# georgeretsi/smirk

Hardware: AMD Instinct MI355X
Metric: faces/sec (encode+FLAME+render+generate) @224x224 (higher is better)
Workload: dtype f32 results; encoder + generator convs as split-fp16 x3 MFMA with f32 accumulate (fp32-class error), FLAME / raster f32

## Files before the change

include/smirk_hip.h:

```cpp
#ifndef SMIRK_HIP_H
#define SMIRK_HIP_H

#include <stddef.h>
#include <stdint.h>

#ifdef __cplusplus
extern "C" {
#endif

#define SMIRK_OK 0
#define SMIRK_ERR_BAD_ARG (-1)
#define SMIRK_ERR_WORKSPACE (-2)
#define SMIRK_ERR_LAUNCH (-3)
#define SMIRK_ERR_UNSUPPORTED (-4)

const char* smirk_strerror(int code);
unsigned smirk_range_flag_peek(void);
void smirk_range_flag_clear(void);

int smirk_abi_version(void);

#define SMIRK_FLAME_KCHUNK 32

typedef struct SmirkFlameModel {
// ... 115 lines not shown
int smirk_pack_generator_input_split16(const float* a, int Ca, const float* b, int Cb, void* out, int B, int H, int W, void* stream);
int smirk_conv1x1_sigmoid_nchw_split16(const void* in, const float* w , const float* bias, float* out,
                                       int B, int H, int W, int C, int Cout, void* stream);

int smirk_maxpool2x2_nhwc(const float* in, float* out, int B, int H, int W, int C, void* stream);
int smirk_nchw_to_nhwc_pad(const float* in, float* out, int B, int Cin, int H, int W, int Cpad, void* stream);
int smirk_pack_generator_input(const float* rendered, const float* masked, float* out, int B, int H, int W, void* stream);
int smirk_conv1x1_sigmoid_nchw(const float* in, const float* w , const float* bias, float* out,
                               int B, int H, int W, int C, int Cout, void* stream);

int smirk_stem_conv_s2(const float* img_nchw, const float* w , const float* scale,
                       const float* shift, float* out, int B, int H, int W, int Cout, void* stream);
int smirk_dwconv3x3(const float* in, const float* w , const float* scale, const float* shift, float* out,
                    int B, int H, int W, int C, int stride, int relu, void* stream);
int smirk_gap_linear(const float* feat, const float* w, const float* bias, float* out, float* ws, int B, int HW, int C, int N,
                     void* stream);
int smirk_stem_conv_s2_split16(const float* img_nchw, const float* w, const float* scale, const float* shift, void* out, int B, int H,
                               int W, int Cout, void* stream);
int smirk_dwconv3x3_split16(const void* in, const float* w , const float* scale, const float* shift, void* out, int B, int H,
                            int W, int C, int stride, int relu, void* stream);
int smirk_gap_linear_split16(const void* feat, const float* w, const float* bias, float* out, float* ws, int B, int HW, int C, int N,
                             void* stream);
int smirk_expression_clamps(float* params, int B, int n_exp, void* stream);

int smirk_mask_face_weights(const float* tverts, const float* normals, const int32_t* faces , const float* face_prob ,
                            int B, int V, int F, float* weights , void* stream);
int smirk_sample_faces(const float* weights, int B, int F, int num, uint64_t seed, uint64_t offset, int32_t* idx, float* bary,
                       void* stream);
int smirk_points_to_pixels(const float* points, int B, int L, int image_size, int64_t* out, void* stream);
int smirk_maxpool_sq(const float* in, float* tmp, float* out, int B, int H, int W, int radius, int complement, void* stream);
int smirk_bernoulli_field(float* out, size_t n, float p, uint64_t seed, uint64_t offset, void* stream);
int smirk_masking_compose(const float* img, const float* mask, const float* rendered_mask, const float* extra_points ,
                          const float* pmask ,
                          const float* keep, const float* noise_mult, int B, int C, int H, int W, int gen_noise,
                          uint64_t seed, uint64_t offset, float* out, void* stream);
int smirk_rendered_mask(const float* rendered_img, int B, int C, int H, int W, float* out, void* stream);
int smirk_scatter_points_mask(const int64_t* points, const int64_t* rbound, int B, int L, int H, int W, float* out, void* stream);
int smirk_transfer_pixels(const float* img, const int64_t* points1, const int64_t* points2, const int64_t* rbound, int B, int C,
                          int L, int H, int W, int32_t* winner_ws, float* out, void* stream);

size_t smirk_mbconv_lds_bytes(int Cin, int mid, int Cout, int stride);
int smirk_mbconv_image_supported(int H, int W, int Cin, int mid, int Cout, int stride);
int smirk_mbconv_image_split16(const void* x, const void* wexp, const float* s1, const float* b1, const float* wdw, const float* s2, const float* b2,
                               const void* wproj, const float* s3, const float* b3, int residual, void* out, int B, int H, int W, int Cin, int mid,
                               int Cout, void* stream);
int smirk_encoder_head_supported(int stem_cout, int kind, int cin, int mid, int cout, int stride, int skip);
int smirk_encoder_head_fused_split16(const float* img, const float* stem_w, const float* stem_scale, const float* stem_shift, const float* dw_w,
                                     const float* dw_scale, const float* dw_shift, const void* pw_w, const float* pw_scale, const float* pw_shift,
                                     int residual, void* out, int B, int H, int W, int stride, void* stream);
int smirk_mbconv_supported(int Cin, int mid, int Cout, int stride);
int smirk_mbconv_fused_split16(const void* x, const void* wexp, const float* s1, const float* b1, const float* wdw, const float* s2,
                               const float* b2, const void* wproj, const float* s3, const float* b3, int residual, void* out,
                               int B, int H, int W, int Cin, int mid, int Cout, int stride, void* stream);

typedef struct SmirkConvLayer {
    const void* w;
    const float* scale;
    const float* shift;
} SmirkConvLayer;

#define SMIRK_GEN_MAX_RES 16
enum { SMIRK_PRECISION_F32 = 0, SMIRK_PRECISION_F16X3 = 1 };

typedef struct SmirkGeneratorWeights {
    int32_t in_channels, out_channels, features, res_blocks;
    int32_t precision;
    int32_t cin_pad;
    SmirkConvLayer enc[5][2];
    SmirkConvLayer res[SMIRK_GEN_MAX_RES][2];
    SmirkConvLayer up[4];
    SmirkConvLayer dec[4][2];
    const float* final_w;
    const float* final_b;
} SmirkGeneratorWeights;

size_t smirk_generator_workspace_bytes(const SmirkGeneratorWeights* w , int B, int H, int W);
int smirk_generator_forward(const SmirkGeneratorWeights* w, const float* a, int Ca, const float* b, int Cb, float* y,
                            int B, int H, int W, void* const* taps, void* ws, size_t ws_bytes, void* stream);

typedef struct SmirkMbBlock {
    int32_t kind, stride, cin, mid, cout, skip;
    SmirkConvLayer pw, dw, pwl;
} SmirkMbBlock;

#define SMIRK_BACKBONE_MAX_BLOCKS 24
typedef struct SmirkBackboneWeights {
    int32_t n_blocks, precision, n_out;
    int32_t clamp_n_exp;
    int32_t stem_cout, feat_ch;
    SmirkConvLayer stem;
    SmirkMbBlock blocks[SMIRK_BACKBONE_MAX_BLOCKS];
    const float* head_w;
    const float* head_b;
} SmirkBackboneWeights;

size_t smirk_backbone_workspace_bytes(const SmirkBackboneWeights* w , int B, int H, int W);
int smirk_backbone_forward(const SmirkBackboneWeights* w, const float* img, int B, int H, int W, float* out, void* feat_out,
                           void* ws, size_t ws_bytes, void* stream);

size_t smirk_train_reduce_workspace_bytes(int C);
int smirk_bn_train_forward_split16(const void* z, size_t M, int C, const float* gamma, const float* beta, const void* residual, int relu, float eps,
                                   float momentum, float* running_mean, float* running_var, long long* num_batches_tracked, float* save_mean,
                                   float* save_var, float* save_invstd, void* y, void* ws, size_t ws_bytes, void* stream);
size_t smirk_conv_stats_rows_max(const SmirkConvDesc* d);
int smirk_conv_igemm_stats_split16(const SmirkConvDesc* d, const void* in0, const void* in1, const void* w, void* out, float* stats, int* rows, int x1, void* stream);
int smirk_bn_train_forward_partials_split16(const void* z, size_t M, int C, const float* gamma, const float* beta, const void* residual, int relu, float eps,
// ... 98 lines not shown
```

smirk_amd/_lib.py:

```python
import ctypes as C
import os

import torch

HERE = os.path.dirname(os.path.abspath(__file__))
LIB_PATH = os.path.join(HERE, "lib", "libsmirk_hip.so")
LIB_PATH = os.environ.get("SMIRK_HIP_LIBRARY", LIB_PATH)
ABI_VERSION = 13
PACK_DEPTHWISE, PACK_STEM, PACK_CONVT2X2 = -3, -27, -2
SMIRK_OK, SMIRK_ERR_BAD_ARG, SMIRK_ERR_WORKSPACE, SMIRK_ERR_LAUNCH, SMIRK_ERR_UNSUPPORTED = 0, -1, -2, -3, -4

_p = C.c_void_p
_i = C.c_int
_sz = C.c_size_t


class SmirkFlameModel(C.Structure):
    _fields_ = [(n, C.c_int32) for n in ("V", "VP", "F", "n_shape", "n_exp", "KP", "n_static", "n_dyn", "n_lut",
                                         "n_full", "n_mp", "_pad")] + \
               [(n, _p) for n in ("dirs", "v_template", "lbs_weights", "jdirs", "jtemplate", "l_eyelid", "r_eyelid",
                                  "faces", "static_faces", "static_bary", "dyn_faces", "dyn_bary", "full_faces",
                                  "full_bary", "mp_faces", "mp_bary")]


class SmirkRenderMesh(C.Structure):
    _fields_ = [(n, C.c_int32) for n in ("V", "Vf", "Ff", "nnz")] + \
               [(n, _p) for n in ("keep", "faces", "nrm_ptr", "nrm_face", "nrm_corner")]


class SmirkConvDesc(C.Structure):
    _fields_ = [(n, C.c_int32) for n in ("B", "H", "W", "C0", "C1", "Cout", "KH", "KW", "stride", "pad_t", "pad_l",
                                         "Ho", "Wo", "pad_mode", "act", "out_mode")]


class SmirkConvLayer(C.Structure):
    _fields_ = [("w", _p), ("scale", _p), ("shift", _p)]


GEN_MAX_RES, BACKBONE_MAX_BLOCKS = 16, 24
PRECISION_F32, PRECISION_F16X3 = 0, 1


class SmirkGeneratorWeights(C.Structure):
    _fields_ = [(n, C.c_int32) for n in ("in_channels", "out_channels", "features", "res_blocks", "precision", "cin_pad")] + \
               [("enc", SmirkConvLayer * 2 * 5), ("res", SmirkConvLayer * 2 * GEN_MAX_RES), ("up", SmirkConvLayer * 4),
                ("dec", SmirkConvLayer * 2 * 4), ("final_w", _p), ("final_b", _p)]


class SmirkMbBlock(C.Structure):
    _fields_ = [(n, C.c_int32) for n in ("kind", "stride", "cin", "mid", "cout", "skip")] + \
               [("pw", SmirkConvLayer), ("dw", SmirkConvLayer), ("pwl", SmirkConvLayer)]


class SmirkBackboneWeights(C.Structure):
    _fields_ = [(n, C.c_int32) for n in ("n_blocks", "precision", "n_out", "clamp_n_exp", "stem_cout", "feat_ch")] + \
               [("stem", SmirkConvLayer), ("blocks", SmirkMbBlock * BACKBONE_MAX_BLOCKS), ("head_w", _p), ("head_b", _p)]


class SmirkProfileRecord(C.Structure):
    _fields_ = [("kernel", C.c_char * 120), ("flop", C.c_double), ("bytes", C.c_double), ("ms", C.c_float), ("_pad", C.c_int32)]


LOSS_MAX_TERMS, LOSS_CHUNK = 8, 4096
LOSS_SQUARE, LOSS_ABS_IMAGE = 0, 1


class SmirkLossTerm(C.Structure):
    _fields_ = [("pred", _p), ("target", _p), ("row_flags", _p)] + \
               [(n, C.c_int32) for n in ("rows", "row_stride", "cols", "kind", "C", "HW")] + \
               [("weight", C.c_float), ("loss_img", _p), ("grad", _p)]


PAD_ZERO, PAD_REFLECT = 0, 1
ACT_NONE, ACT_RELU = 0, 1
OUT_NHWC, OUT_CONVT2X2 = 0, 1

_SIGS = {
    "smirk_strerror": (C.c_char_p, [_i]),
    "smirk_abi_version": (_i, []),
    "smirk_range_flag_peek": (C.c_uint, []),
    "smirk_range_flag_clear": (None, []),
    "smirk_flame_workspace_bytes": (_sz, [C.POINTER(SmirkFlameModel), _i]),
    "smirk_flame_forward": (_i, [C.POINTER(SmirkFlameModel), _i, _p, _i, _p, _i, _p, _p, _p, _p, _p, _p, _p, _p, _p, _p,
                                 _p, _p, _sz, _p]),
    "smirk_flame_backward_workspace_bytes": (_sz, [C.POINTER(SmirkFlameModel), _i]),
    "smirk_flame_backward": (_i, [C.POINTER(SmirkFlameModel), _p, _i, _p, _i, _p, _i] + [_p] * 5 + [_p, _p] + [_p] * 4 + [_p] * 7 +
                             [_p, _sz, _p]),
    "smirk_vertices2landmarks": (_i, [_p, _i, _i, _p, _p, _p, _i, _p, _p]),
    "smirk_render_workspace_bytes": (_sz, [C.POINTER(SmirkRenderMesh), _i, _i, _i]),
    "smirk_render_forward": (_i, [C.POINTER(SmirkRenderMesh), _i, _i, _i, _p, _p, _p, _p, _p, _p, _p, _p, _p, _sz, _p]),
    "smirk_vertex_normals": (_i, [C.POINTER(SmirkRenderMesh), _i, _p, _p, _p]),
    "smirk_mask_face_weights": (_i, [_p, _p, _p, _p, _i, _i, _i, _p, _p]),
    "smirk_sample_faces": (_i, [_p, _i, _i, _i, C.c_uint64, C.c_uint64, _p, _p, _p]),
    "smirk_points_to_pixels": (_i, [_p, _i, _i, _i, _p, _p]),
    "smirk_maxpool_sq": (_i, [_p, _p, _p, _i, _i, _i, _i, _i, _p]),
    "smirk_bernoulli_field": (_i, [_p, _sz, C.c_float, C.c_uint64, C.c_uint64, _p]),
    "smirk_masking_compose": (_i, [_p, _p, _p, _p, _p, _p, _p, _i, _i, _i, _i, _i, C.c_uint64, C.c_uint64, _p, _p]),
    "smirk_render_backward_workspace_bytes": (_sz, [C.POINTER(SmirkRenderMesh), _i, _i, _i]),
    "smirk_render_backward": (_i, [C.POINTER(SmirkRenderMesh), _i, _i, _i, _p, _p, _p, _p, _p, _p, _p, _p, _sz, _p]),
    "smirk_project_landmarks_backward": (_i, [_p, _p, _p, _i, _i, _p, _p, _p]),
    "smirk_encoder_head_supported": (_i, [_i] * 7),
    "smirk_encoder_head_fused_split16": (_i, [_p] * 10 + [_i, _p] + [_i] * 4 + [_p]),
    "smirk_mbconv_image_supported": (_i, [_i] * 6),
    "smirk_mbconv_image_split16": (_i, [_p] * 10 + [_i, _p] + [_i] * 6 + [_p]),
    "smirk_mbconv_lds_bytes": (_sz, [_i, _i, _i, _i]),
    "smirk_mbconv_supported": (_i, [_i, _i, _i, _i]),
    "smirk_mbconv_fused_split16": (_i, [_p] * 10 + [_i, _p] + [_i] * 7 + [_p]),
    "smirk_warp_affine_u8": (_i, [_p, _i, _i, _i, _p, _i, _i, _i, _p, _p, _p]),
    "smirk_resize_linear_u8": (_i, [_p, _i, _i, _i, _i, _i, _i, _p, _p, _p]),
    "smirk_f32_nchw_to_u8_grid": (_i, [_p, _i, _i, _i, _i, _p, _i, _i, _p]),
    "smirk_u8_hwc_to_f32_nchw": (_i, [_p, _i, _i, _i, _i, _p, _p]),
    "smirk_interp_bilinear_f32": (_i, [_p, _i, _i, _i, _i, _i, _p, _p]),
    "smirk_hull_mask": (_i, [_p, _i, _i, _i, _i, _i, _p, _p]),
    "smirk_rendered_mask": (_i, [_p, _i, _i, _i, _i, _p, _p]),
    "smirk_scatter_points_mask": (_i, [_p, _p, _i, _i, _i, _i, _p, _p]),
    "smirk_transfer_pixels": (_i, [_p, _p, _p, _p, _i, _i, _i, _i, _i, _p, _p, _p]),
    "smirk_project_landmarks": (_i, [_p, _p, _i, _i, _p, _p]),
    "smirk_conv_igemm_f32": (_i, [C.POINTER(SmirkConvDesc), _p, _p, _p, _p, _p, _p, _p, _p]),
    "smirk_conv_igemm_f16x3": (_i, [C.POINTER(SmirkConvDesc), _p, _p, _p, _p, _p, _p, _p, _p]),
    "smirk_conv_igemm_f16x1": (_i, [C.POINTER(SmirkConvDesc), _p, _p, _p, _p, _p, _p, _p, _p]),
    "smirk_conv3x3_tail_f16x3": (_i, [C.POINTER(SmirkConvDesc), _p, _p, _p, _p, _p, _p, _p, _p, _i, _p]),
    "smirk_conv3x3_pool_f16x3": (_i, [C.POINTER(SmirkConvDesc), _p, _p, _p, _p, _p, _p, _p, _p]),
    "smirk_enc1_fused_supported": (_i, [_i, _i, _i, _i]),
    "smirk_enc1_fused_split16": (_i, [_p] * 9 + [_i, _i, _i, _p]),
    "smirk_f32_to_split16": (_i, [_p, _p, _sz, _p]),
    "smirk_split16_to_f32": (_i, [_p, _p, _sz, _p]),
    "smirk_maxpool2x2_split16": (_i, [_p, _p, _i, _i, _i, _i, _p]),
    "smirk_split16_range_check": (_i, [_p, _sz, C.c_float, _p, _p]),
    "smirk_pack_generator_input_split16": (_i, [_p, _i, _p, _i, _p, _i, _i, _i, _p]),
    "smirk_conv1x1_sigmoid_nchw_split16": (_i, [_p, _p, _p, _p, _i, _i, _i, _i, _i, _p]),
    "smirk_maxpool2x2_nhwc": (_i, [_p, _p, _i, _i, _i, _i, _p]),
    "smirk_nchw_to_nhwc_pad": (_i, [_p, _p, _i, _i, _i, _i, _i, _p]),
    "smirk_pack_generator_input": (_i, [_p, _p, _p, _i, _i, _i, _p]),
    "smirk_conv1x1_sigmoid_nchw": (_i, [_p, _p, _p, _p, _i, _i, _i, _i, _i, _p]),
    "smirk_stem_conv_s2": (_i, [_p, _p, _p, _p, _p, _i, _i, _i, _i, _p]),
    "smirk_dwconv3x3": (_i, [_p, _p, _p, _p, _p, _i, _i, _i, _i, _i, _i, _p]),
    "smirk_gap_linear": (_i, [_p, _p, _p, _p, _p, _i, _i, _i, _i, _p]),
    "smirk_stem_conv_s2_split16": (_i, [_p, _p, _p, _p, _p, _i, _i, _i, _i, _p]),
    "smirk_dwconv3x3_split16": (_i, [_p, _p, _p, _p, _p, _i, _i, _i, _i, _i, _i, _p]),
    "smirk_gap_linear_split16": (_i, [_p, _p, _p, _p, _p, _i, _i, _i, _i, _p]),
    "smirk_expression_clamps": (_i, [_p, _i, _i, _p]),
    "smirk_generator_workspace_bytes": (_sz, [C.POINTER(SmirkGeneratorWeights), _i, _i, _i]),
    "smirk_generator_forward": (_i, [C.POINTER(SmirkGeneratorWeights), _p, _i, _p, _i, _p, _i, _i, _i, C.POINTER(_p), _p, _sz, _p]),
    "smirk_backbone_workspace_bytes": (_sz, [C.POINTER(SmirkBackboneWeights), _i, _i, _i]),
    "smirk_backbone_forward": (_i, [C.POINTER(SmirkBackboneWeights), _p, _i, _i, _i, _p, _p, _p, _sz, _p]),
    "smirk_train_reduce_workspace_bytes": (_sz, [_i]),
    "smirk_conv_stats_rows_max": (_sz, [C.POINTER(SmirkConvDesc)]),
    "smirk_conv_igemm_stats_split16": (_i, [C.POINTER(SmirkConvDesc), _p, _p, _p, _p, _p, C.POINTER(C.c_int), _i, _p]),
    "smirk_bn_train_forward_partials_split16": (_i, [_p, _sz, _i, _p, _p, _p, _i, C.c_float, C.c_float, _p, _p, _p, _p, _p, _p, _p, _p, _i, _i, _p]),
    "smirk_dwconv3x3_stats_split16": (_i, [_p, _p, _p, _i, _i, _i, _i, _i, _p, C.POINTER(C.c_int), _p]),
    "smirk_bn_train_forward_split16": (_i, [_p, _sz, _i, _p, _p, _p, _i, C.c_float, C.c_float, _p, _p, _p, _p, _p, _p, _p, _p, _sz, _p]),
    "smirk_bn_train_backward_split16": (_i, [_p, _p, _sz, _i, _p, _p, _p, _p, _i, _p, _p, _p, _p, _sz, _p]),
    "smirk_bn_eval_forward_split16": (_i, [_p, _sz, _i, _p, _p, _p, _p, _p, _i, C.c_float, _p, _p, _p, _p]),
    "smirk_bn_eval_backward_split16": (_i, [_p, _p, _sz, _i, _p, _p, _p, _p, _p, _i, _p, _p]),
    "smirk_colsum_split16": (_i, [_p, _sz, _i, _p, _p, _sz, _p]),
    "smirk_maxpool2x2_backward_split16": (_i, [_p, _p, _p, _p, _i, _i, _i, _i, _p]),
    "smirk_reflect_pad1_backward_split16": (_i, [_p, _p, _p, _i, _i, _i, _i, _p]),
    "smirk_space_to_depth2_split16": (_i, [_p, _p, _i, _i, _i, _i, _p]),
    "smirk_conv1x1_sigmoid_backward_split16": (_i, [_p, _p, _p, _p, _p, _i, _i, _i, _i, _i, _p]),
    "smirk_conv_wgrad_set_mode": (_i, [_i]),
# ... 149 lines not shown
```

smirk_amd/csrc/capi.hip:

```cpp
#include <stdlib.h>
#include <string.h>

#include <map>
#include <mutex>
#include <utility>
#include <vector>

#include "common.h"

extern "C" const char* smirk_strerror(int code) {
    switch (code) {
        case SMIRK_OK: return "ok";
        case SMIRK_ERR_BAD_ARG: return "bad argument (null pointer, size or alignment constraint violated)";
        case SMIRK_ERR_WORKSPACE: return "workspace too small (see smirk_*_workspace_bytes)";
        case SMIRK_ERR_LAUNCH: return "HIP kernel launch failed";
        case SMIRK_ERR_UNSUPPORTED: return "configuration not supported by the gfx950 kernels";
        default: return "unknown smirk error";
    }
}

extern "C" int smirk_abi_version(void) { return 13; }

int smirk_switch(SmirkSwitch s) {
    static const char* const names[] = {"SMIRK_IGEMM_HALO", "SMIRK_IGEMM_PP", "SMIRK_CONV_RING", "SMIRK_DISABLE_PATCH_KERNEL", "SMIRK_DISABLE_ENC1_FUSED",
                                        "SMIRK_DISABLE_MBCONV_IMAGE", "SMIRK_DISABLE_MBCONV_TILE", "SMIRK_DISABLE_MBCONV_FUSED",
                                        "SMIRK_DISABLE_ENCODER_HEAD_FUSED", "SMIRK_GEN_SPLIT_CHAINS", "SMIRK_WGRAD_F16"};
    static_assert(sizeof(names) / sizeof(names[0]) == SMIRK_SW_COUNT, "one name per SmirkSwitch");
    const char* e = getenv(names[s]);
    switch (s) {
        case SMIRK_SW_IGEMM_HALO:
        case SMIRK_SW_CONV_RING: return !e || e[0] != '0';
        case SMIRK_SW_IGEMM_PP: return !e ? 1 : e[0] == '0' ? 0 : e[0] == 'a' ? 2 : 1;
        case SMIRK_SW_GEN_SPLIT_CHAINS: return !e ? 0 : e[0] == '0' ? 1 : e[0] == '3' ? 3 : 2;
        case SMIRK_SW_WGRAD_F16: return e ? atoi(e) : SMIRK_WGRAD_F16_DEFAULT;
        default: return e != nullptr;
    }
}

namespace {
std::mutex g_dev_mu;
std::map<std::pair<int, const void*>, size_t> g_lds_raised;
std::map<int, int> g_dev_cus;
}

int smirk_raise_dynamic_lds(const void* kernel, size_t bytes) {
    int dev = 0;
    if (hipGetDevice(&dev) != hipSuccess) { (void)hipGetLastError(); return SMIRK_ERR_LAUNCH; }
    std::lock_guard<std::mutex> lk(g_dev_mu);
    size_t& raised = g_lds_raised[{dev, kernel}];
    if (bytes <= raised) return SMIRK_OK;
    if (hipFuncSetAttribute(kernel, hipFuncAttributeMaxDynamicSharedMemorySize, (int)bytes) != hipSuccess) { (void)hipGetLastError(); return SMIRK_ERR_LAUNCH; }
    raised = bytes;
    return SMIRK_OK;
}

int smirk_device_cus() {
    int dev = 0;
    if (hipGetDevice(&dev) != hipSuccess) { (void)hipGetLastError(); return 256; }
    std::lock_guard<std::mutex> lk(g_dev_mu);
    auto it = g_dev_cus.find(dev);
    if (it != g_dev_cus.end()) return it->second;
    int cus = 0;
    if (hipDeviceGetAttribute(&cus, hipDeviceAttributeMultiprocessorCount, dev) != hipSuccess || cus <= 0) { (void)hipGetLastError(); cus = 256; }
    g_dev_cus[dev] = cus;
    return cus;
}

namespace {
std::once_flag g_range_once;
unsigned* g_range_host = nullptr;
unsigned* g_range_dev = nullptr;
}
unsigned* smirk_range_flag_device_ptr() {
    std::call_once(g_range_once, [] {
// ... 85 lines not shown
```

smirk_amd/csrc/network.hip:

```cpp
#include <sys/syscall.h>
#include <unistd.h>
#include <stdlib.h>

#include "common.h"

namespace {

struct Arena {
    char* base;
    size_t off;
    void* take(size_t bytes) {
        off = smirk_align_up(off, 256);
        void* p = base ? base + off : nullptr;
        off += bytes;
        return p;
    }
};

struct Rot {
    void* slot[3];
    void* pick(const void* a, const void* b) const {
        for (int i = 0; i < 3; ++i)
            if (slot[i] != a && slot[i] != b) return slot[i];
        return nullptr;
    }
};

inline size_t act_bytes(int B, int H, int W, int C) { return (size_t)B * H * W * C * 4; }

struct GenPlan {
    void* x;
    void* e[4];
    Rot rot;
    size_t total;
};

GenPlan plan_generator(const SmirkGeneratorWeights* w, int B, int H, int W, void* ws) {
    Arena a{(char*)ws, 0};
    GenPlan p;
    const int f = w->features;
    p.x = a.take(act_bytes(B, H, W, w->cin_pad));
    for (int l = 0; l < 4; ++l) p.e[l] = a.take(act_bytes(B, H >> l, W >> l, f << l));
    const size_t big = act_bytes(B, H, W, f);
    for (int i = 0; i < 3; ++i) p.rot.slot[i] = a.take(big);
    p.total = smirk_align_up(a.off, 256);
    return p;
}

int conv_call(bool split, const SmirkConvDesc& d, const void* in0, const void* in1, const SmirkConvLayer& L, const void* residual, void* out,
              void* stream) {
    return split ? smirk_conv_igemm_f16x3(&d, in0, in1, L.w, L.scale, L.shift, residual, out, stream)
                 : smirk_conv_igemm_f32(&d, (const float*)in0, (const float*)in1, (const float*)L.w, L.scale, L.shift, (const float*)residual,
                                        (float*)out, stream);
}

SmirkConvDesc desc3x3(int B, int H, int W, int c0, int c1, int cout, bool reflect, bool relu) {
    SmirkConvDesc d;
// ... 284 lines not shown
extern "C" size_t smirk_backbone_workspace_bytes(const SmirkBackboneWeights* w, int B, int H, int W) {
    if (!backbone_args_ok(w, B, H, W)) return 0;
    return plan_backbone(w, B, H, W, nullptr).total;
}

extern "C" int smirk_backbone_forward(const SmirkBackboneWeights* w, const float* img, int B, int H, int W, float* out, void* feat_out,
                                      void* ws, size_t ws_bytes, void* stream) {
    if (!backbone_args_ok(w, B, H, W) || !img || !ws || (w->n_out > 0 && !out) || (w->n_out == 0 && !feat_out)) return SMIRK_ERR_BAD_ARG;
    const BackbonePlan p = plan_backbone(w, B, H, W, ws);
    if (ws_bytes < p.total) return SMIRK_ERR_WORKSPACE;
    const bool split = w->precision == SMIRK_PRECISION_F16X3;
    const bool no_image = smirk_switch(SMIRK_SW_DISABLE_MBCONV_IMAGE);
    const bool no_tile = smirk_switch(SMIRK_SW_DISABLE_MBCONV_TILE);
    const bool no_fuse = smirk_switch(SMIRK_SW_DISABLE_MBCONV_FUSED);
    const bool fuse_ds = false;
    int h = (H + 1) / 2, wd = (W + 1) / 2;
    void* x = p.rot.slot[0];
    int first_block = 0;
    {
        const SmirkMbBlock& b0 = w->blocks[0];
        const bool no_head = smirk_switch(SMIRK_SW_DISABLE_ENCODER_HEAD_FUSED);
        if (split && !no_head && smirk_encoder_head_supported(w->stem_cout, b0.kind, b0.cin, b0.mid, b0.cout, b0.stride, b0.skip)) {
            TRY(smirk_encoder_head_fused_split16(img, (const float*)w->stem.w, w->stem.scale, w->stem.shift, (const float*)b0.dw.w, b0.dw.scale, b0.dw.shift,
                                                 b0.pw.w, b0.pw.scale, b0.pw.shift, b0.skip ? 1 : 0, x, B, H, W, b0.stride, stream));
            h = (h + b0.stride - 1) / b0.stride; wd = (wd + b0.stride - 1) / b0.stride;
            first_block = 1;
        }
    }
    if (!first_block)
    TRY(split ? smirk_stem_conv_s2_split16(img, (const float*)w->stem.w, w->stem.scale, w->stem.shift, x, B, H, W, w->stem_cout, stream)
              : smirk_stem_conv_s2(img, (const float*)w->stem.w, w->stem.scale, w->stem.shift, (float*)x, B, H, W, w->stem_cout, stream));
    auto pointwise = [&](const void* in, int hh, int ww, int cin, int cout, const SmirkConvLayer& L, bool relu, const void* res, void* o) {
        return conv_call(split, desc1x1(B, hh, ww, cin, cout, relu, false), in, nullptr, L, res, o, stream);
    };
    auto depthwise = [&](const void* in, int hh, int ww, int c, int stride, const SmirkConvLayer& L, void* o) {
        return split ? smirk_dwconv3x3_split16(in, (const float*)L.w, L.scale, L.shift, o, B, hh, ww, c, stride, 1, stream)
                     : smirk_dwconv3x3((const float*)in, (const float*)L.w, L.scale, L.shift, (float*)o, B, hh, ww, c, stride, 1, stream);
    };
    int c = first_block ? w->blocks[0].cout : w->stem_cout;
    for (int i = first_block; i < w->n_blocks; ++i) {
        const SmirkMbBlock& b = w->blocks[i];
        if (b.cin != c) return SMIRK_ERR_BAD_ARG;
        const int ho = (h + b.stride - 1) / b.stride, wo = (wd + b.stride - 1) / b.stride;
        const void* res = b.skip ? x : nullptr;
        if (b.kind == 2) {
            void* o = p.rot.pick(x, nullptr);
            TRY(pointwise(x, h, wd, b.cin, b.cout, b.pw, true, nullptr, o));
            x = o;
        } else if (split && !no_fuse && !no_image && !no_tile && b.kind == 1 && b.cin <= 48 && smirk_mbconv_image_supported(h, wd, b.cin, b.mid, b.cout, b.stride)) {
            void* o = p.rot.pick(x, nullptr);
            TRY(smirk_mbconv_image_split16(x, b.pw.w, b.pw.scale, b.pw.shift, (const float*)b.dw.w, b.dw.scale, b.dw.shift, b.pwl.w, b.pwl.scale, b.pwl.shift,
                                           b.skip ? 1 : 0, o, B, h, wd, b.cin, b.mid, b.cout, stream));
            x = o;
        } else if (split && !no_fuse && (b.kind == 1 || fuse_ds) && smirk_mbconv_supported(b.cin, b.mid, b.cout, b.stride)) {
            void* o = p.rot.pick(x, nullptr);
            const SmirkConvLayer& proj = b.kind == 1 ? b.pwl : b.pw;
            TRY(smirk_mbconv_fused_split16(x, b.kind == 1 ? b.pw.w : nullptr, b.kind == 1 ? b.pw.scale : nullptr, b.kind == 1 ? b.pw.shift : nullptr,
                                           (const float*)b.dw.w, b.dw.scale, b.dw.shift, proj.w, proj.scale, proj.shift, b.skip ? 1 : 0, o, B, h, wd,
                                           b.cin, b.mid, b.cout, b.stride, stream));
            x = o;
        } else if (split && !no_fuse && !no_image && b.kind == 1 && smirk_mbconv_image_supported(h, wd, b.cin, b.mid, b.cout, b.stride)) {
            void* o = p.rot.pick(x, nullptr);
            TRY(smirk_mbconv_image_split16(x, b.pw.w, b.pw.scale, b.pw.shift, (const float*)b.dw.w, b.dw.scale, b.dw.shift, b.pwl.w, b.pwl.scale, b.pwl.shift,
                                           b.skip ? 1 : 0, o, B, h, wd, b.cin, b.mid, b.cout, stream));
            x = o;
        } else if (b.kind == 0) {
            void* t = p.rot.pick(x, nullptr);
            TRY(depthwise(x, h, wd, b.cin, b.stride, b.dw, t));
            void* o = p.rot.pick(x, t);
            TRY(pointwise(t, ho, wo, b.cin, b.cout, b.pw, false, res, o));
            x = o;
        } else {
            void* t = p.rot.pick(x, nullptr);
            TRY(pointwise(x, h, wd, b.cin, b.mid, b.pw, true, nullptr, t));
            void* u = p.rot.pick(x, t);
            TRY(depthwise(t, h, wd, b.mid, b.stride, b.dw, u));
            void* o = p.rot.pick(x, u);
            TRY(pointwise(u, ho, wo, b.mid, b.cout, b.pwl, false, res, o));
            x = o;
        }
        h = ho; wd = wo; c = b.cout;
    }
    if (c != w->feat_ch) return SMIRK_ERR_BAD_ARG;
    if (feat_out) (void)hipMemcpyAsync(feat_out, x, act_bytes(B, h, wd, c), hipMemcpyDeviceToDevice, (hipStream_t)stream);
    if (w->n_out == 0) return SMIRK_OK;
    TRY(split ? smirk_gap_linear_split16(x, w->head_w, w->head_b, out, p.pooled, B, h * wd, c, w->n_out, stream)
              : smirk_gap_linear((const float*)x, w->head_w, w->head_b, out, p.pooled, B, h * wd, c, w->n_out, stream));
    if (w->clamp_n_exp >= 0) TRY(smirk_expression_clamps(out, B, w->clamp_n_exp, stream));
    return SMIRK_OK;
}
```

smirk_amd/smirk_encoder.py:

```python
import os

import torch
import torch.nn as nn

from . import _lib as L

BN_EPS = 1e-3
PRECISION = os.environ.get("SMIRK_AMD_ENCODER_PRECISION", "f16x3")
_STREAMS = {}

_ARCH = {
    "tf_mobilenetv3_large_minimal_100": [
        [("ds", 1, 1, 1.0, 16)],
        [("ir", 1, 2, 4.0, 24), ("ir", 1, 1, 3.0, 24)],
        [("ir", 3, 2, 3.0, 40)],
        [("ir", 1, 2, 6.0, 80), ("ir", 1, 1, 2.5, 80), ("ir", 2, 1, 2.3, 80)],
        [("ir", 2, 1, 6.0, 112)],
        [("ir", 3, 2, 6.0, 160)],
        [("cn", 1, 1, 1.0, 960)],
    ],
    "tf_mobilenetv3_small_minimal_100": [
        [("ds", 1, 2, 1.0, 16)],
        [("ir", 1, 2, 4.5, 24), ("ir", 1, 1, 3.67, 24)],
        [("ir", 1, 2, 4.0, 40), ("ir", 2, 1, 6.0, 40)],
# ... 163 lines not shown
        feat = torch.empty(B, (H + 31) // 32, (W + 31) // 32, self.num_features, device=dev) if want_features else None
        nws = lib.smirk_backbone_workspace_bytes(w, B, H, W)
        if nws == 0:
            raise L.SmirkHipError("unsupported backbone configuration / image size (H, W >= 32)")
        ws = self._ws.get(nws, dev)
        L.check(lib.smirk_backbone_forward(w, L.ptr(img), B, H, W, L.ptr(out, allow_none=True), L.ptr(feat, allow_none=True),
                                           L.ptr(ws, torch.uint8), nws, L.stream_ptr()))
        deps = [src] + list(self.parameters()) + ([] if head is None else list(head.parameters()))
        if out is not None:
            out = L.loud_cut("smirk_amd encoder forward", out, deps)
        if feat is not None:
            feat = L.loud_cut("smirk_amd encoder forward", feat, deps)
        return out, feat

    def _pointwise(self, lib, st, x, pk, relu, residual=None):
        w, sc, sh = pk
        B, H, W, C = x.shape
        d = L.SmirkConvDesc()
        d.B, d.H, d.W, d.C0, d.C1, d.Cout = B, H, W, C, 0, w.shape[0]
        d.KH = d.KW = d.stride = 1
        d.pad_t = d.pad_l = 0
        d.Ho, d.Wo, d.pad_mode = H, W, L.PAD_ZERO
        d.act, d.out_mode = (L.ACT_RELU if relu else L.ACT_NONE), L.OUT_NHWC
        out = torch.empty(B, H, W, w.shape[0], device=x.device)
        P = L.ptr
        fn = lib.smirk_conv_igemm_f16x3 if self._split else lib.smirk_conv_igemm_f32
        L.check(fn(d, P(x), None, P(w), P(sc), P(sh), P(residual, allow_none=True), P(out), st))
        return out

    def _depthwise(self, lib, st, x, pk, stride):
        w, sc, sh = pk
        B, H, W, C = x.shape
        out = torch.empty(B, (H + stride - 1) // stride, (W + stride - 1) // stride, C, device=x.device)
        P = L.ptr
        L.check((lib.smirk_dwconv3x3_split16 if self._split else lib.smirk_dwconv3x3)(P(x), P(w), P(sc), P(sh), P(out), B, H, W, C, stride, 1, st))
        return out

    @staticmethod
    def _fusable(lib, cin, pk, blk):
        if blk.kind == "ds":
            return False
        return bool(lib.smirk_mbconv_supported(cin, pk["dw"][0].shape[1], pk["pw" if blk.kind == "ds" else "pwl"][0].shape[0], blk.stride))

    def _fused_block(self, lib, st, x, pk, blk):
        B, H, W, C = x.shape
        P, N = L.ptr, (lambda t: L.ptr(t, allow_none=True))
        if blk.kind == "ds":
            (wd, s2, b2), (wp, s3, b3) = pk["dw"], pk["pw"]
            we = s1 = b1 = None
        else:
            (we, s1, b1), (wd, s2, b2), (wp, s3, b3) = pk["pw"], pk["dw"], pk["pwl"]
        mid, cout, s = wd.shape[1], wp.shape[0], blk.stride
        out = torch.empty(B, (H + s - 1) // s, (W + s - 1) // s, cout, device=x.device)
        L.check(lib.smirk_mbconv_fused_split16(P(x), N(we), N(s1), N(b1), P(wd), P(s2), P(b2), P(wp), P(s3), P(b3), int(bool(blk.skip)),
                                               P(out), B, H, W, C, mid, cout, s, st))
        return out

    def forward(self, img, _taps=None):
        if _taps is None:
            return self.run(img, want_features=True)[1]
        if self.training:
            raise L.SmirkHipError("the per-layer debugging schedule is eval-mode only; train mode runs through the encoders' forward (encoder_train.py)")
        lib, st, P = L.lib(), L.stream_ptr(), self._pack()
        img = L.as_f32c(img)
        B, _, H, W = img.shape
        w, sc, sh = P["stem"]
        x = torch.empty(B, (H + 1) // 2, (W + 1) // 2, 16, device=img.device)
        L.check((lib.smirk_stem_conv_s2_split16 if self._split else lib.smirk_stem_conv_s2)(L.ptr(img), L.ptr(w), L.ptr(sc), L.ptr(sh), L.ptr(x), B, H, W, 16, st))
        fused = self._split and not os.environ.get("SMIRK_DISABLE_MBCONV_FUSED")
        if _taps is not None:
            _taps.append(("stem", x))
        for si, stg in enumerate(self.blocks):
            for bi, blk in enumerate(stg):
                pk = P[(si, bi)]
                if fused and blk.kind in ("ds", "ir") and self._fusable(lib, x.shape[3], pk, blk):
                    x = self._fused_block(lib, st, x, pk, blk)
                elif blk.kind == "ds":
                    y = self._depthwise(lib, st, x, pk["dw"], blk.stride)
                    x = self._pointwise(lib, st, y, pk["pw"], relu=False, residual=x if blk.skip else None)
                elif blk.kind == "ir":
                    y = self._pointwise(lib, st, x, pk["pw"], relu=True)
                    y = self._depthwise(lib, st, y, pk["dw"], blk.stride)
                    x = self._pointwise(lib, st, y, pk["pwl"], relu=False, residual=x if blk.skip else None)
                else:
                    x = self._pointwise(lib, st, x, pk["pw"], relu=True)
                if _taps is not None:
                    _taps.append((f"block{si}.{bi}:{blk.kind}", x))
        return x


def features_f32(backbone, feat):
    if getattr(backbone, "_split", False):
        from .smirk_generator import split16_to_float
        return split16_to_float(feat)
    return feat


def create_backbone(backbone_name, pretrained=True):
    backbone = MobileNetV3Features(backbone_name)
    return backbone, backbone.feature_info[-1]['num_chs']


class PoseEncoder(nn.Module):
    def __init__(self):
        super().__init__()
        self.encoder, feature_dim = create_backbone('tf_mobilenetv3_small_minimal_100')
# ... 84 lines not shown
```

Measured before the change: 10340.

## Add persistent streaming fused MBConv kernel for stride-2 inverted-residual blocks

After: 10250. About the same (-0.9%).

```diff
diff --git a/include/smirk_hip.h b/include/smirk_hip.h
--- a/include/smirk_hip.h
+++ b/include/smirk_hip.h
@@ -191,6 +191,10 @@
 int smirk_mbconv_fused_split16(const void* x, const void* wexp, const float* s1, const float* b1, const float* wdw, const float* s2,
                                const float* b2, const void* wproj, const float* s3, const float* b3, int residual, void* out,
                                int B, int H, int W, int Cin, int mid, int Cout, int stride, void* stream);
+int smirk_mbconv_s2_stream_supported(int Cin, int mid, int Cout);
+int smirk_mbconv_s2_stream_split16(const void* x, const void* wexp, const float* s1, const float* b1, const float* wdw, const float* s2,
+                                   const float* b2, const void* wproj, const float* s3, const float* b3, void* out, int B, int H, int W,
+                                   int Cin, int mid, int Cout, int max_workgroups, void* stream);
 
 typedef struct SmirkConvLayer {
     const void* w;
diff --git a/smirk_amd/_lib.py b/smirk_amd/_lib.py
--- a/smirk_amd/_lib.py
+++ b/smirk_amd/_lib.py
@@ -6,7 +6,7 @@
 HERE = os.path.dirname(os.path.abspath(__file__))
 LIB_PATH = os.path.join(HERE, "lib", "libsmirk_hip.so")
 LIB_PATH = os.environ.get("SMIRK_HIP_LIBRARY", LIB_PATH)
-ABI_VERSION = 13
+ABI_VERSION = 14
 PACK_DEPTHWISE, PACK_STEM, PACK_CONVT2X2 = -3, -27, -2
 SMIRK_OK, SMIRK_ERR_BAD_ARG, SMIRK_ERR_WORKSPACE, SMIRK_ERR_LAUNCH, SMIRK_ERR_UNSUPPORTED = 0, -1, -2, -3, -4
 
@@ -106,6 +106,8 @@
     "smirk_mbconv_lds_bytes": (_sz, [_i, _i, _i, _i]),
     "smirk_mbconv_supported": (_i, [_i, _i, _i, _i]),
     "smirk_mbconv_fused_split16": (_i, [_p] * 10 + [_i, _p] + [_i] * 7 + [_p]),
+    "smirk_mbconv_s2_stream_supported": (_i, [_i, _i, _i]),
+    "smirk_mbconv_s2_stream_split16": (_i, [_p] * 10 + [_p] + [_i] * 7 + [_p]),
     "smirk_warp_affine_u8": (_i, [_p, _i, _i, _i, _p, _i, _i, _i, _p, _p, _p]),
     "smirk_resize_linear_u8": (_i, [_p, _i, _i, _i, _i, _i, _i, _p, _p, _p]),
     "smirk_f32_nchw_to_u8_grid": (_i, [_p, _i, _i, _i, _i, _p, _i, _i, _p]),
diff --git a/smirk_amd/csrc/capi.hip b/smirk_amd/csrc/capi.hip
--- a/smirk_amd/csrc/capi.hip
+++ b/smirk_amd/csrc/capi.hip
@@ -19,7 +19,7 @@
     }
 }
 
-extern "C" int smirk_abi_version(void) { return 13; }
+extern "C" int smirk_abi_version(void) { return 14; }
 
 int smirk_switch(SmirkSwitch s) {
     static const char* const names[] = {"SMIRK_IGEMM_HALO", "SMIRK_IGEMM_PP", "SMIRK_CONV_RING", "SMIRK_DISABLE_PATCH_KERNEL", "SMIRK_DISABLE_ENC1_FUSED",
diff --git a/smirk_amd/csrc/mbconv_s2_stream.hip b/smirk_amd/csrc/mbconv_s2_stream.hip
--- /dev/null
+++ b/smirk_amd/csrc/mbconv_s2_stream.hip
@@ -0,0 +1,350 @@
+#include <stdio.h>
+
+#include "common.h"
+
+typedef _Float16 half8 __attribute__((ext_vector_type(8)));
+
+#define MBS_ES 36
+
+struct MBSArgs {
+    const char* x;
+    const char* wexp;
+    const float *s1, *b1;
+    const float* wdw;
+    const float *s2, *b2;
+    const char* wproj;
+    const float *s3, *b3;
+    char* out;
+    int B, H, W, Cin, mid, Cout, Ho, Wo, pt, pl, cinp, coutp, tiles_x, tiles_y, es_floats, total;
+};
+
+__device__ __forceinline__ void mbs_barrier() {
+    asm volatile("s_waitcnt lgkmcnt(0)" ::: "memory");
+    __builtin_amdgcn_s_barrier();
+    asm volatile("" ::: "memory");
+}
+
+template <int KS, int NCR>
+__global__ __launch_bounds__(256, 3) void mbconv_s2_stream_kernel(MBSArgs a) {
+    SmirkRangeAccS rng;
+    constexpr int S = 2, THO = 4, TWO = 8;
+    constexpr int HI = (THO - 1) * S + 3, WI = (TWO - 1) * S + 3, NH = HI * WI, MH = (NH + 31) / 32 * 32, MO = THO * TWO;
+    constexpr int ES = MBS_ES, DSB = 144;
+    constexpr int P = KS * 4;
+    constexpr int NIT = (MH * P + 255) / 256;
+    constexpr bool WR = NCR > 0;
+    extern __shared__ __attribute__((aligned(16))) char smem[];
+    const int strideX = a.cinp * 4 + 16;
+    const int nchunks = WR ? NCR : (a.mid + 31) / 32, midp = nchunks * 32;
+    char* Xs = smem;
+    float* Es = (float*)(Xs + MH * strideX);
+    char* Ds = (char*)(Es + a.es_floats);
+    float* Wd = (float*)(Ds + MO * DSB);
+    unsigned char* ok = (unsigned char*)(Wd + 13 * midp);
+    float* Os = Es;
+
+    const int tid0 = threadIdx.x;
+    const size_t xrow = (size_t)a.Cin * 4;
+    const int gmax = a.Cin / 8, Preal = a.Cin / 4;
+    const int ntn = a.coutp / 32;
+    const int tpf = a.tiles_x * a.tiles_y;
+    const half8 hz = {0, 0, 0, 0, 0, 0, 0, 0};
+
+    half8 we[WR ? NCR : 1][KS][2];
+    auto load_we = [&](int c, half8 (*dst)[2], int fr, int hb) {
+        const int ch = 32 * c + fr;
+        const char* wrow = a.wexp + (size_t)(ch < a.mid ? ch : 0) * xrow;
+#pragma unroll
+        for (int s = 0; s < KS; ++s) {
+            const int g = 2 * s + hb;
+            const bool v = ch < a.mid && g < gmax;
+            dst[s][0] = v ? *(const half8*)(wrow + g * 32) : hz;
+            dst[s][1] = v ? *(const half8*)(wrow + g * 32 + 16) : hz;
+        }
+    };
+    if constexpr (WR) {
+#pragma unroll
+        for (int c = 0; c < NCR; ++c) load_we(c, we[c], tid0 & 31, (tid0 >> 5) & 1);
+    } else {
+        load_we(0, we[0], tid0 & 31, (tid0 >> 5) & 1);
+    }
+
+    f32x4 xv[NIT];
+    auto halo_load = [&](int tile, int tid) {
+        const int b = tile / tpf, r = tile - b * tpf, ty = r / a.tiles_x, tx = r - ty * a.tiles_x;
+        const int iy0 = ty * THO * S - a.pt, ix0 = tx * TWO * S - a.pl;
+        const char* xb = a.x + (size_t)b * a.H * a.W * xrow;
+#pragma unroll
+        for (int it = 0; it < NIT; ++it) {
+            const int idx = tid + 256 * it, row = idx / P, pc = idx - row * P;
+            const int iy = iy0 + row / WI, ix = ix0 + row % WI;
+            const int yc = min(max(iy, 0), a.H - 1), xc = min(max(ix, 0), a.W - 1), pcc = min(pc, Preal - 1);
+            xv[it] = *(const f32x4*)(xb + ((size_t)yc * a.W + xc) * xrow + pcc * 16);
+        }
+    };
+    auto halo_store = [&](int tile, int tid) {
+        const int b = tile / tpf, r = tile - b * tpf, ty = r / a.tiles_x, tx = r - ty * a.tiles_x;
+        const int iy0 = ty * THO * S - a.pt, ix0 = tx * TWO * S - a.pl;
+#pragma unroll
+        for (int it = 0; it < NIT; ++it) {
+            const int idx = tid + 256 * it, row = idx / P, pc = idx - row * P;
+            if (idx < MH * P) {
+                const int iy = iy0 + row / WI, ix = ix0 + row % WI;
+                const bool inside = row < NH && iy >= 0 && iy < a.H && ix >= 0 && ix < a.W;
+                const f32x4 z = {0.f, 0.f, 0.f, 0.f};
+                *(f32x4*)(Xs + row * strideX + pc * 16) = (inside && pc < Preal) ? xv[it] : z;
+                if (pc == 0) ok[row] = inside ? 1 : 0;
+            }
+        }
+    };
+
+    int tile = blockIdx.x;
+    halo_load(tile, tid0);
+    const int co0 = (tid0 >> 6) * 32 + (tid0 & 31);
+    const float s3 = co0 < a.Cout ? a.s3[min(co0, a.Cout - 1)] : 0.f, b3 = co0 < a.Cout ? a.b3[min(co0, a.Cout - 1)] : 0.f;
+    for (int base = 0; base < 13 * midp; base += 256 * 4) {
+        float cv[4];
+#pragma unroll
+        for (int u = 0; u < 4; ++u) {
+            const int idx = base + 256 * u + tid0, k = min(idx / midp, 12), ch = idx - (idx / midp) * midp, chc = min(ch, a.mid - 1);
+            const float* src = k < 9 ? a.wdw + (size_t)k * a.mid : k == 9 ? a.s2 : k == 10 ? a.b2 : (k == 11 ? a.s1 : a.b1);
+            const float t = src[chc];
+            cv[u] = (idx < 13 * midp && ch < a.mid) ? t : 0.f;
+        }
+#pragma unroll
+        for (int u = 0; u < 4; ++u) {
+            const int idx = base + 256 * u + tid0;
+            if (idx < 13 * midp) Wd[idx] = cv[u];
+        }
+    }
+    halo_store(tile, tid0);
+    mbs_barrier();
+
+    half8 wpre[2][2];
+    auto load_wp = [&](int c, int wave, int co, int hb) {
+        const char* wrow = a.wproj + (size_t)(co < a.Cout ? co : 0) * a.mid * 4;
+#pragma unroll
+        for (int s = 0; s < 2; ++s) {
+            const int kg = min(4 * c + 2 * s + hb, a.mid / 8 - 1);
+            const bool v = wave < ntn && co < a.Cout && (4 * c + 2 * s + hb) * 8 < a.mid;
+            const half8 t0 = *(const half8*)(wrow + kg * 32), t1 = *(const half8*)(wrow + kg * 32 + 16);
+            wpre[s][0] = v ? t0 : hz;
+            wpre[s][1] = v ? t1 : hz;
+        }
+    };
+
+    for (;;) {
+        const int next = tile + (int)gridDim.x;
+        const bool has_next = next < a.total;
+        const int b = tile / tpf, rt = tile - b * tpf, ty = rt / a.tiles_x, tx = rt - ty * a.tiles_x;
+        const int oy0 = ty * THO, ox0 = tx * TWO;
+        int tid = tid0;
+        asm volatile("" : "+v"(tid));
+        const int lane = tid & 63, wave = tid >> 6, fr = lane & 31, hb = lane >> 5, co = wave * 32 + fr;
+
+        unsigned okm[2] = {0u, 0u};
+#pragma unroll
+        for (int i = 0; i < 2; ++i) {
+            const int t = wave + 4 * i;
+            if (t < MH / 32) {
+#pragma unroll
+                for (int r = 0; r < 16; ++r) okm[i] |= (unsigned)ok[t * 32 + mfma32_row(r, lane)] << r;
+            }
+        }
+        if (has_next) halo_load(next, tid);
+
+        f32x16 pacc[2];
+#pragma unroll
+        for (int h = 0; h < 2; ++h)
+#pragma unroll
+            for (int r = 0; r < 16; ++r) pacc[h][r] = 0.f;
+
+        auto chunk = [&](int c, half8 (*wf)[2]) {
+            {
+                const float s1 = Wd[11 * midp + 32 * c + fr], b1 = Wd[12 * midp + 32 * c + fr];
+#pragma unroll
+                for (int ti = 0; ti < 2; ++ti) {
+                    const int t = wave + 4 * ti;
+                    if (t >= MH / 32) break;
+                    f32x16 e0, e1;
+#pragma unroll
+                    for (int r = 0; r < 16; ++r) { e0[r] = 0.f; e1[r] = 0.f; }
+                    const unsigned om = okm[ti];
+                    const char* arow = Xs + (t * 32 + fr) * strideX;
+#pragma unroll
+                    for (int s = 0; s < KS; ++s) {
+                        const int g = 2 * s + hb;
+                        const half8 ah = *(const half8*)(arow + g * 32), al = *(const half8*)(arow + g * 32 + 16);
+                        e0 = __builtin_amdgcn_mfma_f32_32x32x16_f16(ah, wf[s][0], e0, 0, 0, 0);
+                        e1 = __builtin_amdgcn_mfma_f32_32x32x16_f16(ah, wf[s][1], e1, 0, 0, 0);
+                        e1 = __builtin_amdgcn_mfma_f32_32x32x16_f16(al, wf[s][0], e1, 0, 0, 0);
+                    }
+#pragma unroll
+                    for (int r = 0; r < 16; ++r) {
+                        const int row = t * 32 + mfma32_row(r, lane);
+                        if (row < NH) {
+                            const float v = fmaxf((e0[r] + e1[r] * (1.0f / 2048.0f)) * s1 + b1, 0.f);
+                            Es[row * ES + fr] = ((om >> r) & 1u) ? v : 0.f;
+                        }
+                    }
+                }
+                if constexpr (!WR) load_we(c + 1 < nchunks ? c + 1 : 0, we[0], fr, hb);
+            }
+            mbs_barrier();
+            load_wp(c, wave, co, hb);
+            {
+                const int c4 = tid & 7, cb = 32 * c + c4 * 4;
+                const f32x4 s2 = *(const f32x4*)(Wd + 9 * midp + cb), b2 = *(const f32x4*)(Wd + 10 * midp + cb);
+                const int p = tid >> 3, oy = p / TWO, ox = p % TWO;
+                const float* e = Es + ((oy * S) * WI + ox * S) * ES + c4 * 4;
+                f32x4 acc = {0.f, 0.f, 0.f, 0.f};
+#pragma unroll
+                for (int ky = 0; ky < 3; ++ky) {
+#pragma unroll
+                    for (int kx = 0; kx < 3; ++kx) {
+                        const f32x4 v = *(const f32x4*)(e + (ky * WI + kx) * ES);
+                        const f32x4 wk = *(const f32x4*)(Wd + (ky * 3 + kx) * midp + cb);
+#pragma unroll
+                        for (int k = 0; k < 4; ++k) acc[k] = fmaf(v[k], wk[k], acc[k]);
+                    }
+                    __builtin_amdgcn_sched_barrier(0);
+                }
+                typedef _Float16 half4 __attribute__((ext_vector_type(4)));
+                half4 hi, lo;
+#pragma unroll
+                for (int k = 0; k < 4; ++k) {
+                    const float v = fmaxf(acc[k] * s2[k] + b2[k], 0.f);
+                    _Float16 h, l;
+                    smirk_split1(v, h, l);
+                    hi[k] = h; lo[k] = l;
+                }
+                char* d = Ds + p * DSB + (c4 >> 1) * 32 + (c4 & 1) * 8;
+                *(half4*)d = hi;
+                *(half4*)(d + 16) = lo;
+            }
+            mbs_barrier();
+            if (wave < ntn) {
+                const char* arow = Ds + fr * DSB;
+#pragma unroll
+                for (int s = 0; s < 2; ++s) {
+                    const int g = 2 * s + hb;
+                    const half8 ah = *(const half8*)(arow + g * 32), al = *(const half8*)(arow + g * 32 + 16);
+                    pacc[0] = __builtin_amdgcn_mfma_f32_32x32x16_f16(ah, wpre[s][0], pacc[0], 0, 0, 0);
+                    pacc[1] = __builtin_amdgcn_mfma_f32_32x32x16_f16(ah, wpre[s][1], pacc[1], 0, 0, 0);
+                    pacc[1] = __builtin_amdgcn_mfma_f32_32x32x16_f16(al, wpre[s][0], pacc[1], 0, 0, 0);
+                }
+            }
+        };
+        if constexpr (WR) {
+#pragma unroll
+            for (int c = 0; c < NCR; ++c) chunk(c, we[c]);
+        } else {
+            for (int c = 0; c < nchunks; ++c) chunk(c, we[0]);
+        }
+
+        int tid2 = tid0;
+        asm volatile("" : "+v"(tid2));
+        if (has_next) halo_store(next, tid2);
+        const int lane2 = tid2 & 63, wave2 = tid2 >> 6, co2 = wave2 * 32 + (lane2 & 31);
+        if (wave2 < ntn) {
+#pragma unroll
+            for (int r = 0; r < 16; ++r) {
+                const int row = mfma32_row(r, lane2);
+                Os[row * a.coutp + co2] = (pacc[0][r] + pacc[1][r] * (1.0f / 2048.0f)) * s3 + b3;
+            }
+        }
+        mbs_barrier();
+        {
+            const int G = a.Cout / 8;
+            char* ob = a.out + (size_t)b * a.Ho * a.Wo * a.Cout * 4;
+            for (int idx = tid2; idx < MO * G; idx += 256) {
+                const int p = idx / G, g8 = idx - p * G;
+                const int oy = oy0 + p / TWO, ox = ox0 + p % TWO;
+                if (oy >= a.Ho || ox >= a.Wo) continue;
+                float v[8];
+#pragma unroll
+                for (int k = 0; k < 8; ++k) v[k] = Os[p * a.coutp + g8 * 8 + k];
+                half8 hi, lo;
+                rng.see8(v);
+#pragma unroll
+                for (int k = 0; k < 8; ++k) {
+                    _Float16 h, l;
+                    smirk_split1(v[k], h, l);
+                    hi[k] = h; lo[k] = l;
+                }
+                char* o = ob + ((size_t)oy * a.Wo + ox) * a.Cout * 4 + g8 * 32;
+                *(half8*)o = hi;
+                *(half8*)(o + 16) = lo;
+            }
+        }
+        if (!has_next) break;
+        mbs_barrier();
+        tile = next;
+    }
+    rng.commit();
+}
+
+static int mbs_same_pad_lead(int n) {
+    const int o = (n + 1) / 2;
+    int t = (o - 1) * 2 + 3 - n;
+    if (t < 0) t = 0;
+    return t / 2;
+}
+
+static size_t mbs_lds_bytes(int Cin, int mid, int Cout) {
+    const int cinp = (Cin + 15) / 16 * 16, coutp = (Cout + 31) / 32 * 32, midp = (mid + 31) / 32 * 32;
+    const int NH = 153, MH = 160, MO = 32;
+    const size_t es = (size_t)((NH * MBS_ES > MO * coutp) ? NH * MBS_ES : MO * coutp);
+    return (size_t)MH * (cinp * 4 + 16) + es * 4 + (size_t)MO * 144 + (size_t)13 * midp * 4 + MH;
+}
+
+extern "C" int smirk_mbconv_s2_stream_supported(int Cin, int mid, int Cout) {
+    if (Cin % 8 || mid % 8 || Cout % 8 || Cin <= 0 || mid <= 0 || Cout <= 0) return 0;
+    return Cin <= 32 && Cout <= 96 && mbs_lds_bytes(Cin, mid, Cout) <= 64 * 1024;
+}
+
+template <int KS, int NCR>
+static void mbs_launch(const MBSArgs& a, int grid, size_t lds, hipStream_t st) {
+    SMIRK_LAUNCH((mbconv_s2_stream_kernel<KS, NCR>), dim3((unsigned)grid), dim3(256), lds, st, a);
+}
+
+extern "C" int smirk_mbconv_s2_stream_split16(const void* x, const void* wexp, const float* s1, const float* b1, const float* wdw, const float* s2,
+                                              const float* b2, const void* wproj, const float* s3, const float* b3, void* out, int B, int H, int W,
+                                              int Cin, int mid, int Cout, int max_workgroups, void* stream) {
+    if (!x || !wexp || !s1 || !b1 || !wdw || !s2 || !b2 || !wproj || !s3 || !b3 || !out || B <= 0 || H <= 0 || W <= 0 || max_workgroups < 0)
+        return SMIRK_ERR_BAD_ARG;
+    if (!smirk_mbconv_s2_stream_supported(Cin, mid, Cout)) return SMIRK_ERR_UNSUPPORTED;
+    MBSArgs a;
+    a.x = (const char*)x; a.wexp = (const char*)wexp; a.s1 = s1; a.b1 = b1; a.wdw = wdw; a.s2 = s2; a.b2 = b2;
+    a.wproj = (const char*)wproj; a.s3 = s3; a.b3 = b3; a.out = (char*)out;
+    a.B = B; a.H = H; a.W = W; a.Cin = Cin; a.mid = mid; a.Cout = Cout;
+    a.Ho = (H + 1) / 2; a.Wo = (W + 1) / 2;
+    a.pt = mbs_same_pad_lead(H); a.pl = mbs_same_pad_lead(W);
+    a.cinp = (Cin + 15) / 16 * 16; a.coutp = (Cout + 31) / 32 * 32;
+    a.tiles_x = (a.Wo + 7) / 8; a.tiles_y = (a.Ho + 3) / 4;
+    a.es_floats = (153 * MBS_ES > 32 * a.coutp) ? 153 * MBS_ES : 32 * a.coutp;
+    const long long total = (long long)B * a.tiles_x * a.tiles_y;
+    if (total > 0x7fffffffll - 65536) return SMIRK_ERR_BAD_ARG;
+    a.total = (int)total;
+    const size_t lds = mbs_lds_bytes(Cin, mid, Cout);
+    const int by_lds = (int)((size_t)160 * 1024 / lds), per_cu = by_lds < 3 ? by_lds : 3;
+    long long grid = (long long)per_cu * smirk_device_cus();
+    if (max_workgroups > 0 && grid > max_workgroups) grid = max_workgroups;
+    if (grid > total) grid = total;
+    hipStream_t st = (hipStream_t)stream;
+    const int ks = a.cinp / 16, nchunks = (mid + 31) / 32;
+    if (g_smirk_prof_on) {
+        const double pin = (double)B * H * W, pout = (double)B * a.Ho * a.Wo;
+        char nm[64];
+        snprintf(nm, sizeof(nm), "mbconv_s2_stream_kernel<%d>", ks);
+        smirk_prof_next(nm, 2.0 * pin * Cin * mid + 2.0 * pout * mid * 9 + 2.0 * pout * mid * Cout, 4.0 * (pin * Cin + pout * Cout));
+    }
+    if (ks == 1) {
+        if (nchunks == 2) mbs_launch<1, 2>(a, (int)grid, lds, st);
+        else if (nchunks == 3) mbs_launch<1, 3>(a, (int)grid, lds, st);
+        else mbs_launch<1, 0>(a, (int)grid, lds, st);
+    } else {
+        mbs_launch<2, 0>(a, (int)grid, lds, st);
+    }
+    return smirk_launch_status();
+}
diff --git a/smirk_amd/csrc/network.hip b/smirk_amd/csrc/network.hip
--- a/smirk_amd/csrc/network.hip
+++ b/smirk_amd/csrc/network.hip
@@ -3,6 +3,10 @@
 #include <stdlib.h>
 
 #include "common.h"
+
+#ifndef SMIRK_MBCONV_S2_STREAM
+#define SMIRK_MBCONV_S2_STREAM 1
+#endif
 
 namespace {
 
@@ -393,6 +397,11 @@
             TRY(smirk_mbconv_image_split16(x, b.pw.w, b.pw.scale, b.pw.shift, (const float*)b.dw.w, b.dw.scale, b.dw.shift, b.pwl.w, b.pwl.scale, b.pwl.shift,
                                            b.skip ? 1 : 0, o, B, h, wd, b.cin, b.mid, b.cout, stream));
             x = o;
+        } else if (SMIRK_MBCONV_S2_STREAM && split && !no_fuse && b.kind == 1 && b.stride == 2 && smirk_mbconv_s2_stream_supported(b.cin, b.mid, b.cout)) {
+            void* o = p.rot.pick(x, nullptr);
+            TRY(smirk_mbconv_s2_stream_split16(x, b.pw.w, b.pw.scale, b.pw.shift, (const float*)b.dw.w, b.dw.scale, b.dw.shift, b.pwl.w, b.pwl.scale, b.pwl.shift,
+                                               o, B, h, wd, b.cin, b.mid, b.cout, 0, stream));
+            x = o;
         } else if (split && !no_fuse && (b.kind == 1 || fuse_ds) && smirk_mbconv_supported(b.cin, b.mid, b.cout, b.stride)) {
             void* o = p.rot.pick(x, nullptr);
             const SmirkConvLayer& proj = b.kind == 1 ? b.pwl : b.pw;
diff --git a/smirk_amd/smirk_encoder.py b/smirk_amd/smirk_encoder.py
--- a/smirk_amd/smirk_encoder.py
+++ b/smirk_amd/smirk_encoder.py
@@ -239,6 +239,9 @@
             (we, s1, b1), (wd, s2, b2), (wp, s3, b3) = pk["pw"], pk["dw"], pk["pwl"]
         mid, cout, s = wd.shape[1], wp.shape[0], blk.stride
         out = torch.empty(B, (H + s - 1) // s, (W + s - 1) // s, cout, device=x.device)
+        if blk.kind == "ir" and s == 2 and lib.smirk_mbconv_s2_stream_supported(C, mid, cout):
+            L.check(lib.smirk_mbconv_s2_stream_split16(P(x), P(we), P(s1), P(b1), P(wd), P(s2), P(b2), P(wp), P(s3), P(b3), P(out), B, H, W, C, mid, cout, 0, st))
+            return out
         L.check(lib.smirk_mbconv_fused_split16(P(x), N(we), N(s1), N(b1), P(wd), P(s2), P(b2), P(wp), P(s3), P(b3), int(bool(blk.skip)),
                                                P(out), B, H, W, C, mid, cout, s, st))
         return out
```
